# databendlabs/databend

Hardware: AMD Instinct MI355X
Metric: rows/s TPC-H Q1 hash-agg (higher is better)
Workload: dtype i64/i128 decimal

## Files before the change

databend_amd/csrc/gbk_api.h:

```cpp

extern "C" {

int32_t dbhip_group_hash(const dbhip_col* cols, int32_t ncols, int64_t n, uint64_t* out_hashes,
                         void* stream) {
  DBHIP_REQUIRE(cols && ncols >= 1 && ncols <= GB_MAX_KEYS, "dbhip_group_hash: bad column list");
  if (n == 0) return DBHIP_OK;
  DBHIP_REQUIRE(out_hashes, "dbhip_group_hash: NULL out");
  HashCols hc;
  hc.n = ncols;
  for (int k = 0; k < ncols; ++k) {
    if (!key_type_ok(cols[k].type)) {
      set_error("dbhip_group_hash: unsupported type %d", cols[k].type);
      return DBHIP_ERR_INVALID;
    }
    hc.c[k] = to_gbcol(cols[k]);
  }
  hipStream_t s = resolve_stream(stream);
  unsigned long long* bad = (unsigned long long*)scratch(8, 2, s);
  if (!bad) return DBHIP_ERR_HIP;
  DBHIP_CHECK(hipMemsetAsync(bad, 0, 8, s));
  hipLaunchKernelGGL(group_hash_kernel, dim3(grid_for(ceil_div(n, 4), 256, 1024)), dim3(256), 0, s, hc, n, out_hashes, bad);
  DBHIP_LAUNCH_CHECK();
  return DBHIP_OK;
}
// ... 3 lines not shown
                             int64_t initial_capacity, dbhip_groupby** out_host) {
  DBHIP_REQUIRE(out_host && key_types_host, "dbhip_groupby_create: NULL argument");
  dbhip_groupby* g = new (std::nothrow) dbhip_groupby();
  DBHIP_REQUIRE(g, "dbhip_groupby_create: out of host memory");
  memset(g, 0, sizeof(*g));
  int32_t rc = build_layout(key_types_host, key_nullable_host, nkeys, aggs_host, naggs, &g->L);
  if (rc) { delete g; return rc; }
  int64_t cap = 1024;
  while (cap < initial_capacity) cap <<= 1;
  g->hash_mask = ~0ULL;
  g->part_min_rows = 262144;
  g->hint_groups = initial_capacity;
  if (layout_has_wide_minmax(g->L)) { g->part_forbidden = 1; g->part_bits = -1; }
  hipStream_t s = resolve_stream(nullptr);
  if ((rc = alloc_table(g, cap, s))) { delete g; return rc; }
  hipError_t e = hipMalloc((void**)&g->ctrl, 128);
  if (e == hipSuccess) e = hipMemsetAsync(g->ctrl, 0, 128, s);
  if (e == hipSuccess) e = hipStreamSynchronize(s);
  if (e != hipSuccess) {
    (void)dbhip_groupby_destroy(g);
    return hip_fail(e, "dbhip_groupby_create");
  }
  *out_host = g;
  return DBHIP_OK;
}

int32_t dbhip_groupby_debug_set_hash_mask(dbhip_groupby* g, uint64_t mask) {
  DBHIP_REQUIRE(g && g->count_host == 0, "dbhip_groupby_debug_set_hash_mask: table must be empty");
  g->hash_mask = mask;
  return DBHIP_OK;
}

int32_t dbhip_groupby_debug_set_partition_bits(dbhip_groupby* g, int32_t bits) {
  DBHIP_REQUIRE(g && bits <= PT_MAX_BITS, "dbhip_groupby_debug_set_partition_bits: bad argument");
  if (bits > 0) { g->part_bits = bits; g->part_min_rows = 1; g->part_forbidden = 0; }
  else if (bits == 0) { g->part_bits = 0; g->part_min_rows = 262144; g->part_forbidden = 0; }
  else { g->part_bits = -1; g->part_forbidden = 1; g->part_min_rows = 262144; }
// ... 578 lines not shown
  hipLaunchKernelGGL(gb_compact_blocks_kernel, dim3(n_blocks), dim3(256), 0, s, blocks, stride, W, -1, g->rows_in);
  DBHIP_LAUNCH_CHECK();
  return merge_rows(g, g->rows_in, total, s);
}

int32_t dbhip_groupby_reset(dbhip_groupby* g, void* stream) {
  DBHIP_REQUIRE(g, "dbhip_groupby_reset: NULL argument");
  hipStream_t s = resolve_stream(stream);
  if (g->fa_pipe) { const int32_t rc = dbhip_fagg_pipe_reset_internal(g->fa_pipe, s); if (rc) return rc; }
  if (g->cap <= (1 << 20)) {
    hipLaunchKernelGGL(gb_reset_unless_off_kernel, dim3(grid_for(g->cap, 256, 256)), dim3(256), 0, s, (const uint64_t*)nullptr, (int64_t)0, 0, (int64_t)0,
                       g->slot_hash, g->cap, g->ctrl);
    DBHIP_LAUNCH_CHECK();
  } else {
    DBHIP_CHECK(hipMemsetAsync(g->slot_hash, 0, (size_t)g->cap * 8, s));
    DBHIP_CHECK(hipMemsetAsync(g->ctrl, 0, 128, s));
  }
  reset_host_state(g);
  return DBHIP_OK;
}

int32_t dbhip_groupby_destroy(dbhip_groupby* g) {
  if (!g) return DBHIP_OK;
  (void)hipDeviceSynchronize();
  if (g->fa_pipe) dbhip_fagg_pipe_destroy_internal(g->fa_pipe);
  if (g->slot_hash) (void)dbhip_free(g->slot_hash);
  if (g->rows) (void)dbhip_free(g->rows);
  if (g->ctrl) (void)hipFree(g->ctrl);
  if (g->rows_in) (void)dbhip_free(g->rows_in);
  if (g->gid) (void)dbhip_free(g->gid);
  if (g->retry) (void)dbhip_free(g->retry);
  if (g->partial) (void)dbhip_free(g->partial);
  if (g->part_meta) (void)dbhip_free(g->part_meta);
  if (g->spill_idx) (void)dbhip_free(g->spill_idx);
  if (g->spill_rows) (void)dbhip_free(g->spill_rows);
  if (g->gbc_spill) (void)dbhip_free(g->gbc_spill);
  if (g->gbc_split) (void)dbhip_free(g->gbc_split);
  if (g->xcur) (void)hipFree(g->xcur);
  if (g->arena) (void)dbhip_free(g->arena);
  delete g;
  return DBHIP_OK;
}

// ... 3 lines not shown
```

databend_amd/csrc/gbk_merge_lds.h:

```cpp

namespace {

int32_t ensure(void** p, size_t* cap, size_t bytes) {
  if (*cap >= bytes) return DBHIP_OK;
  if (*p) {
    int32_t rc = dbhip_free(*p);
    if (rc) return rc;
    *p = nullptr; *cap = 0;
  }
  size_t want = bytes + (bytes >> 3) + 256;
  int32_t rc = dbhip_alloc(want, p);
  if (rc) { *p = nullptr; return rc; }
  *cap = want;
  return DBHIP_OK;
}

int32_t alloc_table(dbhip_groupby* g, int64_t cap, hipStream_t s) {
  uint64_t* nh = nullptr;
  uint64_t* nr = nullptr;
  int32_t rc = dbhip_alloc((size_t)cap * 8, (void**)&nh);
  if (rc == DBHIP_OK) rc = dbhip_alloc((size_t)cap * g->L.W * 8, (void**)&nr);
  hipError_t e = rc == DBHIP_OK ? hipMemsetAsync(nh, 0, (size_t)cap * 8, s) : hipSuccess;
  if (rc != DBHIP_OK || e != hipSuccess) {
    if (nh) (void)dbhip_free(nh);
// ... 163 lines not shown
                            const uint64_t* n_dev, const uint64_t* abort_dev, int deferred) {
  if (n == 0) return DBHIP_OK;
  if (n > 0xFFFFFFF0LL) {
    set_error("groupby: more than 2^32 rows in one call");
    return DBHIP_ERR_INVALID;
  }
  int32_t rc;
  if ((rc = ensure((void**)&g->gid, &g->gid_cap, (size_t)n * 4))) return rc;
  if ((rc = ensure((void**)&g->retry, &g->retry_cap, (size_t)n * 4))) return rc;
  const int grid = grid_for(n, 256);
  uint64_t* host_ctrl = pinned_words(0);
  if (!host_ctrl) return DBHIP_ERR_HIP;
  const uint64_t* cur_rows = rows_in;
  int64_t cur_n = n;
  const DevCount dc{n_dev, abort_dev};
  if ((deferred || (g->count_host + n) * 135 <= g->cap * 100) && n <= 256) {
    hipLaunchKernelGGL(gb_merge_small_kernel, dim3(1), dim3(256), 0, s, g->L, cur_rows, cur_n, g->slot_hash, g->rows, g->cap, g->hash_mask, g->gid,
                       g->retry, g->ctrl, dc, g->arena);
    DBHIP_LAUNCH_CHECK();
    if (deferred) return DBHIP_OK;
    DBHIP_CHECK(hipMemcpyAsync(host_ctrl, g->ctrl, 5 * sizeof(uint64_t), hipMemcpyDeviceToHost, s));
    DBHIP_CHECK(hipStreamSynchronize(s));
    g->count_host = (int64_t)host_ctrl[0];
    if (host_ctrl[3] & 2) {
      set_error("groupby: a string key longer than 12 bytes was met; keep the CPU operator for this block");
      return DBHIP_ERR_UNSUPPORTED;
    }
    if (host_ctrl[1]) {
      set_error("groupby: collision chain filled the table during retry; create the table with a larger capacity");
      return DBHIP_ERR_CAPACITY;
    }
    return DBHIP_OK;
  }
  if (deferred || (g->count_host + n) * 135 <= g->cap * 100) {
    DBHIP_CHECK(hipMemsetAsync(&g->ctrl[1], 0, 16, s));
    hipLaunchKernelGGL(gb_probe_kernel, dim3(grid), dim3(256), 0, s, g->L, cur_rows, cur_n, g->slot_hash, g->rows, g->cap,
                       g->hash_mask, g->gid, g->ctrl, dc, g->arena);
    if (deferred == 1 || (!deferred && g->count_host > 0 && g->count_host <= 32 && n <= 65536) || n <= 2048 || layout_has_wide_minmax(g->L))
      hipLaunchKernelGGL(gb_accum_lowcard_kernel, dim3(deferred == 1 && grid > 16 ? 16 : grid), dim3(256), 0, s, g->L, cur_rows, cur_n, g->rows, g->gid, g->retry,
                         g->ctrl, dc, g->arena);
    else
      hipLaunchKernelGGL(gb_accum_kernel, dim3(grid), dim3(256), 0, s, g->L, cur_rows, cur_n, g->rows, g->gid, g->retry, g->ctrl, dc, g->arena);
    hipLaunchKernelGGL(gb_retry_kernel, dim3(1), dim3(64), 0, s, g->L, cur_rows, g->slot_hash, g->rows, g->cap, g->hash_mask,
                       g->gid, g->retry, g->ctrl, g->arena);
    DBHIP_LAUNCH_CHECK();
    if (deferred) return DBHIP_OK;
    DBHIP_CHECK(hipMemcpyAsync(host_ctrl, g->ctrl, 5 * sizeof(uint64_t), hipMemcpyDeviceToHost, s));
    DBHIP_CHECK(hipStreamSynchronize(s));
    g->count_host = (int64_t)host_ctrl[0];
    if (host_ctrl[3] & 2) {
      set_error("groupby: a string key longer than 12 bytes was met; keep the CPU operator for this block");
      return DBHIP_ERR_UNSUPPORTED;
    }
    if (host_ctrl[1]) {
      set_error("groupby: collision chain filled the table during retry; create the table with a larger capacity");
      return DBHIP_ERR_CAPACITY;
    }
    return DBHIP_OK;
  }
// ... 27 lines not shown
    DBHIP_CHECK(hipMemcpyAsync(host_ctrl, g->ctrl, 5 * sizeof(uint64_t), hipMemcpyDeviceToHost, s));
    DBHIP_CHECK(hipStreamSynchronize(s));
    g->count_host = (int64_t)host_ctrl[0];
    if (host_ctrl[3] & 2) {
      set_error("groupby: a string key longer than 12 bytes was met; keep the CPU operator for this block");
      return DBHIP_ERR_UNSUPPORTED;
    }
    if (host_ctrl[1] & 2) {
      set_error("groupby: collision chain filled the table during retry; create the table with a larger capacity");
      return DBHIP_ERR_CAPACITY;
    }
    return DBHIP_OK;
  }
  set_error("groupby: table did not converge after repeated growth");
  return DBHIP_ERR_CAPACITY;
}


constexpr int FK_MAXKW = 4;
constexpr int FK_MAXA = 6;
constexpr uint32_t FK_SPILL = 0xFFFFFFFFu;

template <int KW, int NA, bool HI>
struct FkRow {
  uint64_t kw[KW];
  uint64_t h;
  uint64_t aw[NA];
  uint64_t ah[HI ? NA : 1];
  uint32_t avalid;
};
// ... 246 lines not shown
```

databend_amd/csrc/gbk_partitioned.h:

```cpp

namespace {
__device__ __forceinline__ uint32_t part_of(uint64_t h, int pbits) { return (uint32_t)(h >> (64 - pbits)); }
#include "gb_compact.h"

bool gbc_enabled(const dbhip_groupby* g) {
  return !g->gbc_off && g->hash_mask == ~0ULL && !g->has_long;
}

#define GBC_NV_DISPATCH(KW_, nv_, CALL)                                                                          \
  do { if (nv_ == 1) { CALL(KW_, 1); } else if (nv_ == 2) { CALL(KW_, 2); } else if (nv_ == 4) { CALL(KW_, 4); } else { CALL(KW_, 8); } } while (0)
#define GBC_DISPATCH(D, CALL)                                                     \
  do {                                                                            \
    const int nvc_ = gbc_nv_class(D);                                             \
    switch ((D).kw) {                                                             \
      case 1: GBC_NV_DISPATCH(1, nvc_, CALL); break;                              \
      case 2: GBC_NV_DISPATCH(2, nvc_, CALL); break;                              \
      case 3: GBC_NV_DISPATCH(3, nvc_, CALL); break;                              \
      default: GBC_NV_DISPATCH(4, nvc_, CALL); break;                             \
    }                                                                             \
  } while (0)
#define GBC_FOR_ALL(M) M(1, 1) M(1, 2) M(1, 4) M(1, 8) M(2, 1) M(2, 2) M(2, 4) M(2, 8) M(3, 1) M(3, 2) M(3, 4) M(3, 8) M(4, 1) M(4, 2) M(4, 4) M(4, 8)

constexpr int PT_MAX_BITS = 14;
constexpr int PT_PMAX = 1 << PT_MAX_BITS;
// ... 116 lines not shown
    const int64_t tile_rows = (int64_t)threads * R;
    const int64_t cn = n - *done < limit ? n - *done : limit;
    const int64_t ntiles = ceil_div(cn, tile_rows);
    int grid = (int)(ntiles < max_grid_i ? ntiles : max_grid_i);
    if (!gbc && !g->fast_trusted && ntiles >= 64) {
      const int64_t gmax = probing ? ntiles / 4 : ntiles / 8;
      if (grid > gmax) grid = (int)gmax;
    }
    const int64_t tpb = ceil_div(ntiles, grid);
    grid = (int)ceil_div(ntiles, tpb);
    if ((rc = ensure((void**)&g->partial, &g->partial_cap, (size_t)grid * lcap_i * L.W * 8))) return rc;
    int64_t spill_cap = cn;
    if (g->fast_trusted && cn > (4 << 20)) spill_cap = cn / 64 > (4 << 20) ? cn / 64 : (4 << 20);
    if ((rc = ensure((void**)&g->rows_in, &g->rows_in_cap, (size_t)spill_cap * L.W * 8))) return rc;
    DBHIP_CHECK(hipMemsetAsync(&g->ctrl[5], 0, 16, s));
    FkArgs A;
    A.spill_cap = (uint64_t)spill_cap;
    A.row0 = *done; A.n = cn; A.tiles_per_block = tpb; A.lcap = lcap_i; A.sw = sw;
    A.llimit = (uint32_t)(lcap_i - lcap_i / 4);
    A.hash_mask = g->hash_mask; A.partial = g->partial; A.spill = g->rows_in; A.ctrl = g->ctrl;
    if (gbc) {
      static std::once_flag gbc_attr_once;
      static hipError_t gbc_attr_err = hipSuccess;
      std::call_once(gbc_attr_once, [] {
#define GBC_RAISE(KW_, NV_) if (gbc_attr_err == hipSuccess) gbc_attr_err = hipFuncSetAttribute((const void*)gbc_agg_kernel<KW_, NV_, true>, hipFuncAttributeMaxDynamicSharedMemorySize, 150 * 1024);
        GBC_FOR_ALL(GBC_RAISE)
#undef GBC_RAISE
      });
      DBHIP_CHECK(gbc_attr_err);
      GbcAggArgs G;
// ... 841 lines not shown
    hipLaunchKernelGGL((gb_part_scatter_kernel<2>), dim3((int)nwg), dim3(T), lds2, s, L, C, row0, cn, pbits, rows_per_wg, mat,
                       g->rows_in, g->ctrl);
  else if (lds1 <= lds_max)
    hipLaunchKernelGGL((gb_part_scatter_kernel<1>), dim3((int)nwg), dim3(T), lds1, s, L, C, row0, cn, pbits, rows_per_wg, mat,
                       g->rows_in, g->ctrl);
  else
    hipLaunchKernelGGL((gb_part_scatter_kernel<0>), dim3((int)nwg), dim3(T), (size_t)P * 4, s, L, C, row0, cn, pbits,
                       rows_per_wg, mat, g->rows_in, g->ctrl);
  DBHIP_LAUNCH_CHECK();
  return DBHIP_OK;
}

int32_t add_chunk_partitioned(dbhip_groupby* g, const GbCols& C, int64_t row0, int64_t cn, hipStream_t s,
                              int64_t* spilled) {
  const GbLayout& L = g->L;
  const int pbits = g->part_bits;
  const int P = 1 << pbits;
  int lcap, sw;
  size_t lds_bytes;
  int32_t rc;
  GbcDesc D;
  const bool gbc = g->gbc_active && !g->gbc_skip && !g->part_direct && gbc_enabled(g) && gbc_describe(L, C, &D);
  D.ctrl = g->ctrl;
  if (!gbc) g->gbc_active = 0;
  table_geometry(g, &lcap, &sw, &lds_bytes);
  if (gbc) rc = gbc_partition_scatter(g, C, D, row0, cn, pbits, s);
  else rc = partition_scatter(g, C, row0, cn, pbits, s);
  if (rc) return rc;
  if (!gbc && (rc = ensure((void**)&g->spill_idx, &g->spill_idx_cap, (size_t)cn * 4))) return rc;
  uint32_t* base = g->part_meta + PT_PMAX;
// ... 213 lines not shown
```

databend_amd/csrc/gbk_rows.h:

```cpp

namespace {

struct HashCols {
  GbCol c[GB_MAX_KEYS];
  int n;
};

__global__ __launch_bounds__(256) void group_hash_kernel(HashCols hc, int64_t n, uint64_t* out,
                                                         unsigned long long* bad) {
  constexpr int U = 4;
  const int64_t T = (int64_t)gridDim.x * blockDim.x;
  const int64_t t = (int64_t)blockIdx.x * blockDim.x + threadIdx.x;
  for (int64_t base = 0; base < n; base += U * T) {
    int64_t row[U];
    bool in[U];
    uint64_t h[U];
#pragma unroll
    for (int u = 0; u < U; ++u) {
      row[u] = base + u * T + t;
      in[u] = row[u] < n;
      if (!in[u]) row[u] = n - 1;
      h[u] = 0;
    }
    for (int k = 0; k < hc.n; ++k) {
// ... 450 lines not shown
        for (int a = 0; a < L.naggs; ++a) gb_atomic_merge(L, a, d + L.agg_off[a], r + L.agg_off[a]);
        done = true;
      }
      pos = (pos + 1) & cmask;
    }
    if (!done) ctrl[1] |= 2;
  }
}
__global__ void gb_retry_kernel(GbLayout L, const uint64_t* rows_in, uint64_t* slot_hash, uint64_t* rows,
                                int64_t cap, uint64_t hash_mask, const uint32_t* gid,
                                const uint32_t* retry, uint64_t* ctrl, uint8_t* arena) {
  if (threadIdx.x != 0 || blockIdx.x != 0) return;
  gb_retry_body(L, rows_in, slot_hash, rows, cap, hash_mask, gid, retry, ctrl, arena);
}

__global__ __launch_bounds__(256) void gb_merge_small_kernel(GbLayout L, const uint64_t* rows_in, int64_t n, uint64_t* slot_hash, uint64_t* rows,
                                                             int64_t cap, uint64_t hash_mask, uint32_t* gid, uint32_t* retry, uint64_t* ctrl,
                                                             DevCount dc, uint8_t* arena) {
  n = dev_rows(dc, n);
  if (threadIdx.x < 2) ctrl[1 + threadIdx.x] = 0;
  __threadfence();
  __syncthreads();
  gb_probe_body(L, rows_in, n, slot_hash, rows, cap, hash_mask, gid, ctrl, arena);
  __threadfence();
  __syncthreads();
  gb_accum_lowcard_body(L, rows_in, n, rows, gid, retry, ctrl, arena);
  __threadfence();
  __syncthreads();
  if (threadIdx.x == 0) gb_retry_body(L, rows_in, slot_hash, rows, cap, hash_mask, gid, retry, ctrl, arena);
}

__global__ __launch_bounds__(256) void gb_rehash_kernel(GbLayout L, const uint64_t* old_hash,
                                                        const uint64_t* old_rows, int64_t old_cap,
                                                        uint64_t* new_hash, uint64_t* new_rows,
                                                        int64_t new_cap, uint64_t hash_mask) {
  const uint64_t cmask = (uint64_t)new_cap - 1;
  for (int64_t s = (int64_t)blockIdx.x * blockDim.x + threadIdx.x; s < old_cap;
       s += (int64_t)gridDim.x * blockDim.x) {
    uint64_t hw = old_hash[s];
    if (hw == 0) continue;
    const uint64_t* r = old_rows + s * L.W;
    uint64_t pos = home_slot(probe_word(r[L.hash_word], hash_mask), new_cap);
    while (true) {
      unsigned long long old = atomicCAS((unsigned long long*)&new_hash[pos], 0ULL, (unsigned long long)hw);
// ... 71 lines not shown
  uint64_t off = 0;
  for (int p = 0; p < b; ++p)
    if (p != skip) off += blocks[(int64_t)p * stride_words];
  const uint64_t* src = blocks + (int64_t)b * stride_words + W;
  uint64_t* dst = out + off * W;
  for (uint64_t i = threadIdx.x; i < cnt * (uint64_t)W; i += blockDim.x) dst[i] = src[i];
}

__global__ __launch_bounds__(256) void gb_reset_unless_off_kernel(const uint64_t* __restrict__ blocks, int64_t stride_words, int n_blocks,
                                                                  int64_t max_rows, uint64_t* __restrict__ slot_hash, int64_t cap, uint64_t* __restrict__ ctrl) {
  for (int p = 0; p < n_blocks; ++p) {
    const uint64_t c = blocks[(int64_t)p * stride_words];
    if (c == ~0ULL || (int64_t)c > max_rows || blocks[(int64_t)p * stride_words + 1] != 0) return;
  }
  for (int64_t i = (int64_t)blockIdx.x * blockDim.x + threadIdx.x; i < cap; i += (int64_t)gridDim.x * blockDim.x) slot_hash[i] = 0;
  if (blockIdx.x == 0 && threadIdx.x < 16) ctrl[threadIdx.x] = 0;
}

struct ResultPtrs {
  void* keys[GB_MAX_KEYS];
  uint32_t* key_validity[GB_MAX_KEYS];
  void* aggs[GB_MAX_AGGS];
  uint32_t* agg_validity[GB_MAX_AGGS];
  uint64_t* hashes;
  const uint8_t* arena;
};

__device__ __forceinline__ bool gb_sum256_out_of_range(const uint64_t* s) {
  const bool neg = (s[3] >> 63) != 0;
  if (s[4] != (neg ? ~0ULL : 0ULL)) return true;
  uint64_t m[4] = {s[0], s[1], s[2], s[3]};
// ... 399 lines not shown
```

databend_amd/csrc/k_fagg.hip:

```cpp
#include "fagg_device.h"
#include "runtime.h"

#include <dirent.h>
#include <dlfcn.h>
#include <errno.h>
#include <sys/stat.h>
#include <fcntl.h>
#include <signal.h>
#include <spawn.h>
#include <sys/wait.h>
#include <unistd.h>

#include <atomic>
#include <chrono>
#include <deque>
#include <map>
#include <mutex>
#include <string>

#include <stdlib.h>
#include <string.h>
#include <time.h>

using namespace dbhip;

int32_t dbhip_groupby_merge_rows_dev_internal(dbhip_groupby* g, const uint64_t* rows, int64_t n_max, const uint64_t* n_dev,
                                              const uint64_t* abort_dev, hipStream_t s);
int32_t dbhip_groupby_merge_rows_internal(dbhip_groupby* g, const uint64_t* rows, int64_t n, hipStream_t s);
int64_t dbhip_groupby_capacity_internal(dbhip_groupby* g);
int32_t dbhip_groupby_reserve_merge_internal(dbhip_groupby* g, int64_t n);
int64_t dbhip_groupby_count_internal(dbhip_groupby* g);
const GbLayout* dbhip_groupby_layout_internal(dbhip_groupby* g);
int32_t dbhip_groupby_merge_rows_deferred_internal(dbhip_groupby* g, const uint64_t* rows, int64_t n_max, const uint64_t* n_dev,
                                                   const uint64_t* abort_dev, hipStream_t s);
int32_t dbhip_groupby_ensure_room_internal(dbhip_groupby* g, int64_t extra, hipStream_t s);
uint64_t* dbhip_groupby_ctrl_internal(dbhip_groupby* g);
void dbhip_groupby_set_count_internal(dbhip_groupby* g, int64_t count);
void** dbhip_groupby_pipe_slot_internal(dbhip_groupby* g);

namespace {

#include "build/jit_embed.inc"
// ... 898 lines not shown
  if (rc) return rc;
  A.filter_bits = filter_bitmap; A.filter_off = filter_bit_offset; A.n = n;
  A.has_filter = filter_bitmap != nullptr;
  const size_t lds = (size_t)(A.P.n_slots > 6 ? A.P.n_slots : 6) * FA_ROWS * 256 * 8;
  if (lds > 60 * 1024) {
    set_error("dbhip_groupby_add_block_program: %d live LDS slots exceed the register file; split the expression", A.P.n_slots);
    return DBHIP_ERR_UNSUPPORTED;
  }
  const int64_t nchunks = ceil_div(n, 64 * FA_ROWS);
  const int grid = (int)(ceil_div(nchunks, 4) < 512 ? ceil_div(nchunks, 4) : 512);
  if (FaPipe* pp = (FaPipe*)*dbhip_groupby_pipe_slot_internal(g); pp && !t_prepare_only) {
    int64_t committed = 0;
    if ((rc = fa_pipe_checkpoint(g, pp, &committed, true))) return rc;
  }
  const size_t rows_bytes = (size_t)grid * FA_MAX_SLOTS * L.W * 8;
  uint8_t* ws = (uint8_t*)scratch(rows_bytes + 64, 6, s);
  if (!ws) return DBHIP_ERR_HIP;
  uint64_t* ctrl = (uint64_t*)ws;
  A.ctrl = ctrl;
  A.partial_rows = (uint64_t*)(ws + 64);
  A.P.err_words = nullptr;
  A.P.err_count = (unsigned long long*)&ctrl[2];
  uint64_t* host_ctrl = pinned_words(1);
  if (!host_ctrl) return DBHIP_ERR_HIP;
  host_ctrl[0] = host_ctrl[1] = host_ctrl[2] = 0;
  const int64_t n_max = (int64_t)grid * FA_MAX_SLOTS;
  const bool chained = (dbhip_groupby_count_internal(g) + n_max) * 135 <= dbhip_groupby_capacity_internal(g) * 100;
  if ((rc = dbhip_groupby_reserve_merge_internal(g, n_max))) return rc;
  if (t_prepare_only) {
    (void)jit_kernel(A, dbhip_groupby_count_internal(g) > 4 ? 8 : 4, general, nwords, JIT_COMPILE);
    if (FaPipe* pq = (FaPipe*)*dbhip_groupby_pipe_slot_internal(g); pq && pq->on)
      (void)jit_kernel(A, dbhip_groupby_count_internal(g) > 4 ? 8 : 4, general, nwords, JIT_COMPILE, nullptr, true);
    return DBHIP_OK;
  }
  for (int variant = dbhip_groupby_count_internal(g) > 4 ? 1 : 0; variant < 2; ++variant) {
    DBHIP_CHECK(hipMemsetAsync(ctrl, 0, 64, s));
    kernel_timer_start(s);
    if ((rc = fa_launch(A, variant == 0 ? 4 : 8, general, nwords, grid, lds, s))) return rc;
    kernel_timer_stop(s);
    DBHIP_LAUNCH_CHECK();
    DBHIP_CHECK(hipMemcpyAsync(host_ctrl, ctrl, 24, hipMemcpyDeviceToHost, s));
    if (chained && !may_raise) {
      rc = dbhip_groupby_merge_rows_dev_internal(g, A.partial_rows, n_max, &ctrl[0], &ctrl[1], s);
      if (rc) return rc;
      if (!(host_ctrl[1] & 3)) return DBHIP_OK;
    } else {
      DBHIP_CHECK(hipStreamSynchronize(s));
    }
    if (!(host_ctrl[1] & 1)) break;
  }
  if (host_ctrl[1] & 2) {
    set_error("dbhip_groupby_add_block_program: a group key string is longer than 12 bytes");
    return DBHIP_ERR_UNSUPPORTED;
  }
  if (host_ctrl[1] & 1) {
    set_error("dbhip_groupby_add_block_program: more than %d distinct groups inside one workgroup; use the operator-at-a-time path", FA_MAX_SLOTS);
    return DBHIP_ERR_CAPACITY;
  }
  if (host_ctrl[2]) {
    set_error("dbhip_groupby_add_block_program: %llu row error(s) in the fused maps (Decimal overflow / divided by zero); "
              "evaluate the maps with dbhip_expr_eval to get the rows", (unsigned long long)host_ctrl[2]);
    return DBHIP_ERR_ROW_ERRORS;
  }
// ... 105 lines not shown
      if (inputs[c].data == col.data && inputs[c].type == col.type && inputs[c].validity == col.validity &&
          inputs[c].validity_offset == col.validity_offset && inputs[c].is_scalar == col.is_scalar) found = c;
    if (found < 0) {
      if (n_inputs >= EX_MAX_INPUTS) return DBHIP_ERR_UNSUPPORTED;
      if (col.type == DBHIP_T_DEC128) { int wide = 0; for (int c = 0; c < n_inputs; ++c) wide += inputs[c].type == DBHIP_T_DEC128; if (wide >= 2) return DBHIP_ERR_UNSUPPORTED; }
      inputs[n_inputs] = col;
      found = n_inputs++;
    }
    arg_regs[a] = DBHIP_ARG_INPUT(found);
    any_arg = true;
  }
  if (!any_arg) return DBHIP_ERR_UNSUPPORTED;
  dbhip_agg_program prog;
  prog.prog = nullptr; prog.n_ins = 0; prog.inputs = inputs; prog.n_inputs = n_inputs; prog.filter_reg = -1; prog.arg_regs = arg_regs;
  t_jit_only = true; t_jit_pending = false; t_jit_may_compile = may_compile;
  const int32_t rc = dbhip_groupby_add_block_program(g, keys, &prog, n, C.filter, C.filter_off + row0, (void*)s);
  t_jit_only = false;
  return rc;
}
int32_t dbhip_fagg_pipe_add_columns_internal(dbhip_groupby* g, void* pipe, const GbCols& C, int64_t n, hipStream_t s) {
  FaPipe* pp = (FaPipe*)pipe;
  if (!pp || !pp->on || pp->given_up || jit_mode() == 0) return -1;
  const GbLayout& L = *dbhip_groupby_layout_internal(g);
  if (!dbhip_fagg_layout_ok_internal(L)) return -1;
  dbhip_col keys[FA_KW], inputs[EX_MAX_INPUTS];
  int32_t arg_regs[FA_MAXA];
  int n_inputs = 0;
  for (int k = 0; k < L.nkeys; ++k)
    if (!fa_offset_col(C.key[k], 0, &keys[k])) return -1;
  bool any_arg = false;
// ... 74 lines not shown
```

databend_amd/csrc/k_groupby.hip:

```cpp
#include <mutex>
#include "gb_device.h"
#include "runtime.h"

#include <math.h>
#include <stdlib.h>
#include <string.h>

#include <new>
#include <vector>

using namespace dbhip;

#define GB_INVALID_SLOT 0xFFFFFFFFu

struct dbhip_groupby {
  int64_t hint_groups;
  GbLayout L;
  int64_t cap;
  uint64_t* slot_hash;
  uint64_t* rows;
  uint64_t* ctrl;
  uint64_t hash_mask;
  int64_t count_host;
  uint64_t* rows_in; size_t rows_in_cap;
// ... 18 lines not shown
  int has_long;
  uint64_t* xcur;
  int xcur_dirty;
  int fagg_disabled;
  int gbc_off;
  int gbc_active;
  int gbc_lcap;
  int gbc_nodirect;
  int gbc_part_lcap_max;
  uint32_t gbc_part_cap;
  uint64_t* gbc_spill; size_t gbc_spill_cap;
  uint64_t arena_pinned, arena_live;
  int gbc_skip;
  uint32_t* gbc_split; size_t gbc_split_cap;
  void* fa_pipe;
};

int32_t dbhip_fagg_pipe_drain_internal(dbhip_groupby* g, void* pipe, hipStream_t s);
void dbhip_fagg_pipe_destroy_internal(void* pipe);
int32_t dbhip_fagg_pipe_reset_internal(void* pipe, hipStream_t s);
struct GbCols;
int32_t dbhip_fagg_pipe_add_columns_internal(dbhip_groupby* g, void* pipe, const GbCols& C, int64_t n, hipStream_t s);
#define GB_DRAIN(g, s)                                                                   \
  do {                                                                                   \
    if ((g) && (g)->fa_pipe) {                                                           \
      const int32_t _rc = dbhip_fagg_pipe_drain_internal((g), (g)->fa_pipe, (s));        \
      if (_rc) return _rc;                                                               \
    }                                                                                    \
  } while (0)

#include "gbk_rows.h"
int32_t dbhip_groupby_build_layout_internal(const int32_t* key_types, const uint8_t* key_nullable, int nkeys, const dbhip_agg_desc* aggs,
                                            int naggs, GbLayout* L) {
  return build_layout(key_types, key_nullable, nkeys, aggs, naggs, L);
}
#include "gbk_merge_lds.h"
int32_t dbhip_fagg_add_columns_internal(dbhip_groupby* g, const GbCols& C, int64_t row0, int64_t n, bool may_compile, hipStream_t s);
bool dbhip_fagg_last_refusal_is_pending_internal();
#include "gbk_partitioned.h"

int32_t dbhip_groupby_merge_rows_internal(dbhip_groupby* g, const uint64_t* rows, int64_t n, hipStream_t s) {
  return merge_rows(g, rows, n, s);
}
int32_t dbhip_groupby_merge_rows_dev_internal(dbhip_groupby* g, const uint64_t* rows, int64_t n_max, const uint64_t* n_dev,
                                              const uint64_t* abort_dev, hipStream_t s) {
  return merge_rows(g, rows, n_max, s, n_dev, abort_dev);
}
int32_t dbhip_groupby_reserve_merge_internal(dbhip_groupby* g, int64_t n) {
  int32_t rc;
  if ((rc = ensure((void**)&g->gid, &g->gid_cap, (size_t)n * 4))) return rc;
  return ensure((void**)&g->retry, &g->retry_cap, (size_t)n * 4);
}
int32_t dbhip_groupby_merge_rows_deferred_internal(dbhip_groupby* g, const uint64_t* rows, int64_t n_max, const uint64_t* n_dev,
                                                   const uint64_t* abort_dev, hipStream_t s) {
  return merge_rows_unpinned(g, rows, n_max, s, n_dev, abort_dev, 1);
}
int32_t dbhip_groupby_ensure_room_internal(dbhip_groupby* g, int64_t extra, hipStream_t s) {
  uint64_t cnt = 0;
  DBHIP_CHECK(hipMemcpyAsync(&cnt, &g->ctrl[0], 8, hipMemcpyDeviceToHost, s));
  DBHIP_CHECK(hipStreamSynchronize(s));
  g->count_host = (int64_t)cnt;
  while ((g->count_host + extra) * 135 > g->cap * 100) {
// ... 14 lines not shown
```

databend_amd/csrc/k_q1.hip:

```cpp
#include "gb_device.h"
#include "runtime.h"

#include <stdlib.h>
#include <string.h>

using namespace dbhip;

int32_t dbhip_groupby_merge_rows_internal(dbhip_groupby* g, const uint64_t* rows, int64_t n, hipStream_t s);
int32_t dbhip_groupby_merge_rows_dev_internal(dbhip_groupby* g, const uint64_t* rows, int64_t n_max, const uint64_t* n_dev,
                                              const uint64_t* abort_dev, hipStream_t s);
int64_t dbhip_groupby_capacity_internal(dbhip_groupby* g);
int64_t dbhip_groupby_count_internal(dbhip_groupby* g);
const GbLayout* dbhip_groupby_layout_internal(dbhip_groupby* g);

namespace {

constexpr int MAX_SLOTS = 8;
constexpr int Q1_W = 15;

struct alignas(16) U4 {
  uint32_t x, y, z, w;
};
struct alignas(16) L2 {
  int64_t a, b;
};
// ... 282 lines not shown
                   L->key_type[1] == DBHIP_T_STRING && L->agg_off[0] == 5 && L->agg_off[2] == 7 &&
                   L->agg_off[5] == 14 && L->agg_words[2] == 3 && L->agg_words[3] == 3;
  DBHIP_REQUIRE(layout_ok, "dbhip_q1_fused: table was not created by dbhip_q1_create_groupby");
  if (n == 0) return DBHIP_OK;
  DBHIP_REQUIRE(l_quantity && l_extendedprice && l_discount && l_tax && l_returnflag_views &&
                    l_linestatus_views && l_shipdate,
                "dbhip_q1_fused: NULL column");
  uintptr_t al = (uintptr_t)l_quantity | (uintptr_t)l_extendedprice | (uintptr_t)l_discount |
                 (uintptr_t)l_tax | (uintptr_t)l_returnflag_views | (uintptr_t)l_linestatus_views;
  DBHIP_REQUIRE((al & 15) == 0 && ((uintptr_t)l_shipdate & 7) == 0,
                "dbhip_q1_fused: columns must be 16-byte aligned (shipdate 8-byte)");
  hipStream_t s = resolve_stream(stream);
  const int64_t ntiles = ceil_div(n, 128);
  const int grid = (int)(ceil_div(ntiles, 4) < 512 ? ceil_div(ntiles, 4) : 512);
  size_t rows_bytes = (size_t)grid * MAX_SLOTS * Q1_W * 8;
  uint8_t* ws = (uint8_t*)scratch(rows_bytes + 64, 4, s);
  if (!ws) return DBHIP_ERR_HIP;
  uint64_t* ctrl = (uint64_t*)ws;
  uint64_t* partial = (uint64_t*)(ws + 64);
  Q1Args A;
  A.qty = l_quantity; A.price = l_extendedprice; A.disc = l_discount; A.tax = l_tax;
  A.rf = (const U4*)l_returnflag_views; A.ls = (const U4*)l_linestatus_views;
  A.shipdate = l_shipdate; A.cutoff = shipdate_cutoff; A.n = n;
  A.partial_rows = partial; A.ctrl = ctrl;
  uint64_t* host_ctrl = pinned_words(1);
  if (!host_ctrl) return DBHIP_ERR_HIP;
  host_ctrl[0] = host_ctrl[1] = 0;
  const int64_t n_max4 = (int64_t)grid * 4, n_max8 = (int64_t)grid * MAX_SLOTS;
  const bool chained = (dbhip_groupby_count_internal(g) + n_max8) * 135 <= dbhip_groupby_capacity_internal(g) * 100;
  for (int variant = 0; variant < 2; ++variant) {
    DBHIP_CHECK(hipMemsetAsync(ctrl, 0, 64, s));
    kernel_timer_start(s);
    if (variant == 0) hipLaunchKernelGGL(q1_fused_kernel, dim3(grid), dim3(256), 0, s, A);
    else hipLaunchKernelGGL(q1_fused_kernel_8slots, dim3(grid), dim3(256), 0, s, A);
    kernel_timer_stop(s);
    DBHIP_LAUNCH_CHECK();
    DBHIP_CHECK(hipMemcpyAsync(host_ctrl, ctrl, 16, hipMemcpyDeviceToHost, s));
    if (chained) {
      int32_t rc = dbhip_groupby_merge_rows_dev_internal(g, partial, variant == 0 ? n_max4 : n_max8, &ctrl[0], &ctrl[1], s);
      if (rc) return rc;
      if (!(host_ctrl[1] & 3)) return DBHIP_OK;
    } else {
      DBHIP_CHECK(hipStreamSynchronize(s));
    }
    if (!(host_ctrl[1] & 1)) break;
  }
  if (host_ctrl[1] & 2) {
    set_error("dbhip_q1_fused: a group key string is longer than 12 bytes; use the operator-at-a-time path");
    return DBHIP_ERR_UNSUPPORTED;
  }
  if (host_ctrl[1] & 1) {
    set_error("dbhip_q1_fused: more than %d distinct groups inside one workgroup; use the operator-at-a-time path", MAX_SLOTS);
    return DBHIP_ERR_CAPACITY;
  }
  return dbhip_groupby_merge_rows_internal(g, partial, (int64_t)host_ctrl[0], s);
}

}
```

Measured before the change: 91.63 billion.

## Publish fused-merge outcome through mapped host record and skip redundant ctrl memsets

The fused Q1 and fagg paths now keep their control words inside the group-by ctrl block. The closing merge kernel writes the counts and flags into a host-mapped pinned record tagged with a sequence number. This replaces the separate device-to-host memcpy of ctrl words, and the per-call memsets are skipped when the ctrl words are known to be clean after the previous call. The change adds tail_clean bookkeeping on every path that touches ctrl, plus system-scope atomics in the retry kernel. Any path that misses marking the state dirty could leave stale flags behind.

Result: no change. 90.99 billion (median of 2 runs) (-0.7%).

```diff
diff --git a/databend_amd/csrc/gbk_api.h b/databend_amd/csrc/gbk_api.h
--- a/databend_amd/csrc/gbk_api.h
+++ b/databend_amd/csrc/gbk_api.h
@@ -41,13 +41,14 @@
   if (layout_has_wide_minmax(g->L)) { g->part_forbidden = 1; g->part_bits = -1; }
   hipStream_t s = resolve_stream(nullptr);
   if ((rc = alloc_table(g, cap, s))) { delete g; return rc; }
-  hipError_t e = hipMalloc((void**)&g->ctrl, 128);
-  if (e == hipSuccess) e = hipMemsetAsync(g->ctrl, 0, 128, s);
+  hipError_t e = hipMalloc((void**)&g->ctrl, GB_CTRL_WORDS * 8);
+  if (e == hipSuccess) e = hipMemsetAsync(g->ctrl, 0, GB_CTRL_WORDS * 8, s);
   if (e == hipSuccess) e = hipStreamSynchronize(s);
   if (e != hipSuccess) {
     (void)dbhip_groupby_destroy(g);
     return hip_fail(e, "dbhip_groupby_create");
   }
+  g->tail_clean = 1;
   *out_host = g;
   return DBHIP_OK;
 }
@@ -656,8 +657,9 @@
     DBHIP_LAUNCH_CHECK();
   } else {
     DBHIP_CHECK(hipMemsetAsync(g->slot_hash, 0, (size_t)g->cap * 8, s));
-    DBHIP_CHECK(hipMemsetAsync(g->ctrl, 0, 128, s));
-  }
+    DBHIP_CHECK(hipMemsetAsync(g->ctrl, 0, GB_CTRL_WORDS * 8, s));
+  }
+  g->tail_clean = 1;
   reset_host_state(g);
   return DBHIP_OK;
 }
@@ -669,6 +671,7 @@
   if (g->slot_hash) (void)dbhip_free(g->slot_hash);
   if (g->rows) (void)dbhip_free(g->rows);
   if (g->ctrl) (void)hipFree(g->ctrl);
+  if (g->tail_host) (void)hipHostFree(g->tail_host);
   if (g->rows_in) (void)dbhip_free(g->rows_in);
   if (g->gid) (void)dbhip_free(g->gid);
   if (g->retry) (void)dbhip_free(g->retry);
diff --git a/databend_amd/csrc/gbk_merge_lds.h b/databend_amd/csrc/gbk_merge_lds.h
--- a/databend_amd/csrc/gbk_merge_lds.h
+++ b/databend_amd/csrc/gbk_merge_lds.h
@@ -201,9 +201,11 @@
   const uint64_t* cur_rows = rows_in;
   int64_t cur_n = n;
   const DevCount dc{n_dev, abort_dev};
+  const bool closing = deferred == 3;
+  if (!closing) g->tail_clean = 0;
   if ((deferred || (g->count_host + n) * 135 <= g->cap * 100) && n <= 256) {
     hipLaunchKernelGGL(gb_merge_small_kernel, dim3(1), dim3(256), 0, s, g->L, cur_rows, cur_n, g->slot_hash, g->rows, g->cap, g->hash_mask, g->gid,
-                       g->retry, g->ctrl, dc, g->arena);
+                       g->retry, g->ctrl, dc, g->arena, closing ? g->tail_dev : (uint64_t*)nullptr, g->tail_seq);
     DBHIP_LAUNCH_CHECK();
     if (deferred) return DBHIP_OK;
     DBHIP_CHECK(hipMemcpyAsync(host_ctrl, g->ctrl, 5 * sizeof(uint64_t), hipMemcpyDeviceToHost, s));
@@ -220,16 +222,20 @@
     return DBHIP_OK;
   }
   if (deferred || (g->count_host + n) * 135 <= g->cap * 100) {
-    DBHIP_CHECK(hipMemsetAsync(&g->ctrl[1], 0, 16, s));
+    if (!closing) DBHIP_CHECK(hipMemsetAsync(&g->ctrl[1], 0, 16, s));
     hipLaunchKernelGGL(gb_probe_kernel, dim3(grid), dim3(256), 0, s, g->L, cur_rows, cur_n, g->slot_hash, g->rows, g->cap,
                        g->hash_mask, g->gid, g->ctrl, dc, g->arena);
-    if (deferred == 1 || (!deferred && g->count_host > 0 && g->count_host <= 32 && n <= 65536) || n <= 2048 || layout_has_wide_minmax(g->L))
+    if (deferred == 1 || ((!deferred || closing) && g->count_host > 0 && g->count_host <= 32 && n <= 65536) || n <= 2048 || layout_has_wide_minmax(g->L))
       hipLaunchKernelGGL(gb_accum_lowcard_kernel, dim3(deferred == 1 && grid > 16 ? 16 : grid), dim3(256), 0, s, g->L, cur_rows, cur_n, g->rows, g->gid, g->retry,
                          g->ctrl, dc, g->arena);
     else
       hipLaunchKernelGGL(gb_accum_kernel, dim3(grid), dim3(256), 0, s, g->L, cur_rows, cur_n, g->rows, g->gid, g->retry, g->ctrl, dc, g->arena);
-    hipLaunchKernelGGL(gb_retry_kernel, dim3(1), dim3(64), 0, s, g->L, cur_rows, g->slot_hash, g->rows, g->cap, g->hash_mask,
-                       g->gid, g->retry, g->ctrl, g->arena);
+    if (closing)
+      hipLaunchKernelGGL(gb_retry_close_kernel, dim3(1), dim3(64), 0, s, g->L, cur_rows, g->slot_hash, g->rows, g->cap, g->hash_mask,
+                         g->gid, g->retry, g->ctrl, g->arena, g->tail_dev, g->tail_seq);
+    else
+      hipLaunchKernelGGL(gb_retry_kernel, dim3(1), dim3(64), 0, s, g->L, cur_rows, g->slot_hash, g->rows, g->cap, g->hash_mask,
+                         g->gid, g->retry, g->ctrl, g->arena);
     DBHIP_LAUNCH_CHECK();
     if (deferred) return DBHIP_OK;
     DBHIP_CHECK(hipMemcpyAsync(host_ctrl, g->ctrl, 5 * sizeof(uint64_t), hipMemcpyDeviceToHost, s));
@@ -287,6 +293,60 @@
   }
   set_error("groupby: table did not converge after repeated growth");
   return DBHIP_ERR_CAPACITY;
+}
+
+int32_t fused_begin(dbhip_groupby* g, bool chained, hipStream_t s) {
+  if (chained && !g->tail_host) {
+    uint64_t* host = nullptr;
+    uint64_t* dev = nullptr;
+    DBHIP_CHECK(hipHostMalloc((void**)&host, GB_REC_WORDS * sizeof(uint64_t), hipHostMallocMapped));
+    memset(host, 0, GB_REC_WORDS * sizeof(uint64_t));
+    const hipError_t e = hipHostGetDevicePointer((void**)&dev, host, 0);
+    if (e != hipSuccess || !dev) {
+      (void)hipHostFree(host);
+      return hip_fail(e != hipSuccess ? e : hipErrorInvalidValue, "groupby: mapping the outcome record");
+    }
+    g->tail_host = host;
+    g->tail_dev = dev;
+  }
+  if (!g->tail_clean) {
+    DBHIP_CHECK(hipMemsetAsync(&g->ctrl[GB_CTRL_FUSED], 0, 24, s));
+    if (chained) DBHIP_CHECK(hipMemsetAsync(&g->ctrl[1], 0, 16, s));
+  }
+  g->tail_clean = 0;
+  return DBHIP_OK;
+}
+int32_t fused_finish(dbhip_groupby* g, const uint64_t* rows, int64_t n_max, bool chained, hipStream_t s, uint64_t* out) {
+  uint64_t* fused = g->ctrl + GB_CTRL_FUSED;
+  if (!chained) {
+    uint64_t* host = pinned_words(1);
+    if (!host) return DBHIP_ERR_HIP;
+    DBHIP_CHECK(hipMemcpyAsync(host, fused, 24, hipMemcpyDeviceToHost, s));
+    DBHIP_CHECK(hipStreamSynchronize(s));
+    out[0] = host[0]; out[1] = host[1]; out[2] = host[2];
+    return DBHIP_OK;
+  }
+  ++g->tail_seq;
+  int32_t rc = merge_rows_unpinned(g, rows, n_max, s, &fused[0], &fused[1], 3);
+  if (rc) return rc;
+  DBHIP_CHECK(hipStreamSynchronize(s));
+  const uint64_t* rec = g->tail_host;
+  if (__atomic_load_n(&rec[GB_REC_SEQ], __ATOMIC_ACQUIRE) != g->tail_seq) {
+    set_error("groupby: the outcome record of the merge behind a fused kernel is not the one of this call");
+    return DBHIP_ERR_HIP;
+  }
+  g->tail_clean = 1;
+  out[0] = rec[GB_REC_FUSED_ROWS]; out[1] = rec[GB_REC_FUSED_FLAGS]; out[2] = rec[GB_REC_FUSED_ERRORS];
+  g->count_host = (int64_t)rec[GB_REC_COUNT];
+  if (rec[GB_REC_ERROR] & 2) {
+    set_error("groupby: a string key longer than 12 bytes was met; keep the CPU operator for this block");
+    return DBHIP_ERR_UNSUPPORTED;
+  }
+  if (rec[GB_REC_OVERFLOW]) {
+    set_error("groupby: collision chain filled the table during retry; create the table with a larger capacity");
+    return DBHIP_ERR_CAPACITY;
+  }
+  return pin_string_states(g, s);
 }
 
 
diff --git a/databend_amd/csrc/gbk_partitioned.h b/databend_amd/csrc/gbk_partitioned.h
--- a/databend_amd/csrc/gbk_partitioned.h
+++ b/databend_amd/csrc/gbk_partitioned.h
@@ -154,6 +154,7 @@
     if (g->fast_trusted && cn > (4 << 20)) spill_cap = cn / 64 > (4 << 20) ? cn / 64 : (4 << 20);
     if ((rc = ensure((void**)&g->rows_in, &g->rows_in_cap, (size_t)spill_cap * L.W * 8))) return rc;
     DBHIP_CHECK(hipMemsetAsync(&g->ctrl[5], 0, 16, s));
+    g->tail_clean = 0;
     FkArgs A;
     A.spill_cap = (uint64_t)spill_cap;
     A.row0 = *done; A.n = cn; A.tiles_per_block = tpb; A.lcap = lcap_i; A.sw = sw;
@@ -1025,6 +1026,7 @@
 int32_t add_chunk_partitioned(dbhip_groupby* g, const GbCols& C, int64_t row0, int64_t cn, hipStream_t s,
                               int64_t* spilled) {
   const GbLayout& L = g->L;
+  g->tail_clean = 0;
   const int pbits = g->part_bits;
   const int P = 1 << pbits;
   int lcap, sw;
diff --git a/databend_amd/csrc/gbk_rows.h b/databend_amd/csrc/gbk_rows.h
--- a/databend_amd/csrc/gbk_rows.h
+++ b/databend_amd/csrc/gbk_rows.h
@@ -488,9 +488,30 @@
   gb_retry_body(L, rows_in, slot_hash, rows, cap, hash_mask, gid, retry, ctrl, arena);
 }
 
+constexpr int GB_CTRL_WORDS = 32;
+constexpr int GB_CTRL_FUSED = 16;
+enum { GB_REC_COUNT = 0, GB_REC_OVERFLOW, GB_REC_ERROR, GB_REC_FUSED_ROWS, GB_REC_FUSED_FLAGS, GB_REC_FUSED_ERRORS, GB_REC_SEQ, GB_REC_WORDS };
+__device__ __forceinline__ void gb_close_tail(uint64_t* ctrl, uint64_t* rec, uint64_t seq) {
+  const int src[GB_REC_SEQ] = {0, 1, 3, GB_CTRL_FUSED, GB_CTRL_FUSED + 1, GB_CTRL_FUSED + 2};
+#pragma unroll
+  for (int q = 0; q < GB_REC_SEQ; ++q)
+    __hip_atomic_store(&rec[q], __hip_atomic_load(&ctrl[src[q]], __ATOMIC_RELAXED, __HIP_MEMORY_SCOPE_AGENT), __ATOMIC_RELAXED, __HIP_MEMORY_SCOPE_SYSTEM);
+  ctrl[1] = 0; ctrl[2] = 0;
+  ctrl[GB_CTRL_FUSED] = 0; ctrl[GB_CTRL_FUSED + 1] = 0; ctrl[GB_CTRL_FUSED + 2] = 0;
+  __hip_atomic_store(&rec[GB_REC_SEQ], seq, __ATOMIC_RELEASE, __HIP_MEMORY_SCOPE_SYSTEM);
+  __threadfence_system();
+}
+__global__ void gb_retry_close_kernel(GbLayout L, const uint64_t* rows_in, uint64_t* slot_hash, uint64_t* rows,
+                                      int64_t cap, uint64_t hash_mask, const uint32_t* gid,
+                                      const uint32_t* retry, uint64_t* ctrl, uint8_t* arena, uint64_t* rec, uint64_t seq) {
+  if (threadIdx.x != 0 || blockIdx.x != 0) return;
+  gb_retry_body(L, rows_in, slot_hash, rows, cap, hash_mask, gid, retry, ctrl, arena);
+  gb_close_tail(ctrl, rec, seq);
+}
+
 __global__ __launch_bounds__(256) void gb_merge_small_kernel(GbLayout L, const uint64_t* rows_in, int64_t n, uint64_t* slot_hash, uint64_t* rows,
                                                              int64_t cap, uint64_t hash_mask, uint32_t* gid, uint32_t* retry, uint64_t* ctrl,
-                                                             DevCount dc, uint8_t* arena) {
+                                                             DevCount dc, uint8_t* arena, uint64_t* rec = nullptr, uint64_t seq = 0) {
   n = dev_rows(dc, n);
   if (threadIdx.x < 2) ctrl[1 + threadIdx.x] = 0;
   __threadfence();
@@ -501,7 +522,10 @@
   gb_accum_lowcard_body(L, rows_in, n, rows, gid, retry, ctrl, arena);
   __threadfence();
   __syncthreads();
-  if (threadIdx.x == 0) gb_retry_body(L, rows_in, slot_hash, rows, cap, hash_mask, gid, retry, ctrl, arena);
+  if (threadIdx.x == 0) {
+    gb_retry_body(L, rows_in, slot_hash, rows, cap, hash_mask, gid, retry, ctrl, arena);
+    if (rec) gb_close_tail(ctrl, rec, seq);
+  }
 }
 
 __global__ __launch_bounds__(256) void gb_rehash_kernel(GbLayout L, const uint64_t* old_hash,
@@ -603,7 +627,7 @@
     if (c == ~0ULL || (int64_t)c > max_rows || blocks[(int64_t)p * stride_words + 1] != 0) return;
   }
   for (int64_t i = (int64_t)blockIdx.x * blockDim.x + threadIdx.x; i < cap; i += (int64_t)gridDim.x * blockDim.x) slot_hash[i] = 0;
-  if (blockIdx.x == 0 && threadIdx.x < 16) ctrl[threadIdx.x] = 0;
+  if (blockIdx.x == 0 && threadIdx.x < GB_CTRL_WORDS) ctrl[threadIdx.x] = 0;
 }
 
 struct ResultPtrs {
diff --git a/databend_amd/csrc/k_fagg.hip b/databend_amd/csrc/k_fagg.hip
--- a/databend_amd/csrc/k_fagg.hip
+++ b/databend_amd/csrc/k_fagg.hip
@@ -24,8 +24,11 @@
 
 using namespace dbhip;
 
-int32_t dbhip_groupby_merge_rows_dev_internal(dbhip_groupby* g, const uint64_t* rows, int64_t n_max, const uint64_t* n_dev,
-                                              const uint64_t* abort_dev, hipStream_t s);
+uint64_t* dbhip_groupby_fused_ctrl_internal(dbhip_groupby* g);
+int32_t dbhip_groupby_fused_begin_internal(dbhip_groupby* g, bool chained, hipStream_t s);
+int32_t dbhip_groupby_fused_finish_internal(dbhip_groupby* g, const uint64_t* rows, int64_t n_max, bool chained, hipStream_t s,
+                                            uint64_t* out_host);
+void dbhip_groupby_tail_dirty_internal(dbhip_groupby* g);
 int32_t dbhip_groupby_merge_rows_internal(dbhip_groupby* g, const uint64_t* rows, int64_t n, hipStream_t s);
 int64_t dbhip_groupby_capacity_internal(dbhip_groupby* g);
 int32_t dbhip_groupby_reserve_merge_internal(dbhip_groupby* g, int64_t n);
@@ -954,16 +957,14 @@
     if ((rc = fa_pipe_checkpoint(g, pp, &committed, true))) return rc;
   }
   const size_t rows_bytes = (size_t)grid * FA_MAX_SLOTS * L.W * 8;
-  uint8_t* ws = (uint8_t*)scratch(rows_bytes + 64, 6, s);
+  uint8_t* ws = (uint8_t*)scratch(rows_bytes, 6, s);
   if (!ws) return DBHIP_ERR_HIP;
-  uint64_t* ctrl = (uint64_t*)ws;
+  uint64_t* ctrl = dbhip_groupby_fused_ctrl_internal(g);
   A.ctrl = ctrl;
-  A.partial_rows = (uint64_t*)(ws + 64);
+  A.partial_rows = (uint64_t*)ws;
   A.P.err_words = nullptr;
   A.P.err_count = (unsigned long long*)&ctrl[2];
-  uint64_t* host_ctrl = pinned_words(1);
-  if (!host_ctrl) return DBHIP_ERR_HIP;
-  host_ctrl[0] = host_ctrl[1] = host_ctrl[2] = 0;
+  uint64_t host_ctrl[3] = {0, 0, 0};
   const int64_t n_max = (int64_t)grid * FA_MAX_SLOTS;
   const bool chained = (dbhip_groupby_count_internal(g) + n_max) * 135 <= dbhip_groupby_capacity_internal(g) * 100;
   if ((rc = dbhip_groupby_reserve_merge_internal(g, n_max))) return rc;
@@ -973,20 +974,15 @@
       (void)jit_kernel(A, dbhip_groupby_count_internal(g) > 4 ? 8 : 4, general, nwords, JIT_COMPILE, nullptr, true);
     return DBHIP_OK;
   }
+  const bool queued = chained && !may_raise;
   for (int variant = dbhip_groupby_count_internal(g) > 4 ? 1 : 0; variant < 2; ++variant) {
-    DBHIP_CHECK(hipMemsetAsync(ctrl, 0, 64, s));
+    if ((rc = dbhip_groupby_fused_begin_internal(g, queued, s))) return rc;
     kernel_timer_start(s);
     if ((rc = fa_launch(A, variant == 0 ? 4 : 8, general, nwords, grid, lds, s))) return rc;
     kernel_timer_stop(s);
     DBHIP_LAUNCH_CHECK();
-    DBHIP_CHECK(hipMemcpyAsync(host_ctrl, ctrl, 24, hipMemcpyDeviceToHost, s));
-    if (chained && !may_raise) {
-      rc = dbhip_groupby_merge_rows_dev_internal(g, A.partial_rows, n_max, &ctrl[0], &ctrl[1], s);
-      if (rc) return rc;
-      if (!(host_ctrl[1] & 3)) return DBHIP_OK;
-    } else {
-      DBHIP_CHECK(hipStreamSynchronize(s));
-    }
+    if ((rc = dbhip_groupby_fused_finish_internal(g, A.partial_rows, n_max, queued, s, host_ctrl))) return rc;
+    if (queued && !(host_ctrl[1] & 3)) return DBHIP_OK;
     if (!(host_ctrl[1] & 1)) break;
   }
   if (host_ctrl[1] & 2) {
@@ -1122,6 +1118,7 @@
   dbhip_agg_program prog;
   prog.prog = nullptr; prog.n_ins = 0; prog.inputs = inputs; prog.n_inputs = n_inputs; prog.filter_reg = -1; prog.arg_regs = arg_regs;
   t_jit_only = true; t_jit_pending = false; t_jit_may_compile = may_compile;
+  dbhip_groupby_tail_dirty_internal(g);
   const int32_t rc = dbhip_groupby_add_block_program(g, keys, &prog, n, C.filter, C.filter_off + row0, (void*)s);
   t_jit_only = false;
   return rc;
diff --git a/databend_amd/csrc/k_groupby.hip b/databend_amd/csrc/k_groupby.hip
--- a/databend_amd/csrc/k_groupby.hip
+++ b/databend_amd/csrc/k_groupby.hip
@@ -56,6 +56,9 @@
   int gbc_skip;
   uint32_t* gbc_split; size_t gbc_split_cap;
   void* fa_pipe;
+  int tail_clean;
+  uint64_t tail_seq;
+  uint64_t* tail_host; uint64_t* tail_dev;
 };
 
 int32_t dbhip_fagg_pipe_drain_internal(dbhip_groupby* g, void* pipe, hipStream_t s);
@@ -84,10 +87,13 @@
 int32_t dbhip_groupby_merge_rows_internal(dbhip_groupby* g, const uint64_t* rows, int64_t n, hipStream_t s) {
   return merge_rows(g, rows, n, s);
 }
-int32_t dbhip_groupby_merge_rows_dev_internal(dbhip_groupby* g, const uint64_t* rows, int64_t n_max, const uint64_t* n_dev,
-                                              const uint64_t* abort_dev, hipStream_t s) {
-  return merge_rows(g, rows, n_max, s, n_dev, abort_dev);
+uint64_t* dbhip_groupby_fused_ctrl_internal(dbhip_groupby* g) { return g->ctrl + GB_CTRL_FUSED; }
+int32_t dbhip_groupby_fused_begin_internal(dbhip_groupby* g, bool chained, hipStream_t s) { return fused_begin(g, chained, s); }
+int32_t dbhip_groupby_fused_finish_internal(dbhip_groupby* g, const uint64_t* rows, int64_t n_max, bool chained, hipStream_t s,
+                                            uint64_t* out_host) {
+  return fused_finish(g, rows, n_max, chained, s, out_host);
 }
+void dbhip_groupby_tail_dirty_internal(dbhip_groupby* g) { g->tail_clean = 0; }
 int32_t dbhip_groupby_reserve_merge_internal(dbhip_groupby* g, int64_t n) {
   int32_t rc;
   if ((rc = ensure((void**)&g->gid, &g->gid_cap, (size_t)n * 4))) return rc;
diff --git a/databend_amd/csrc/k_q1.hip b/databend_amd/csrc/k_q1.hip
--- a/databend_amd/csrc/k_q1.hip
+++ b/databend_amd/csrc/k_q1.hip
@@ -7,8 +7,10 @@
 using namespace dbhip;
 
 int32_t dbhip_groupby_merge_rows_internal(dbhip_groupby* g, const uint64_t* rows, int64_t n, hipStream_t s);
-int32_t dbhip_groupby_merge_rows_dev_internal(dbhip_groupby* g, const uint64_t* rows, int64_t n_max, const uint64_t* n_dev,
-                                              const uint64_t* abort_dev, hipStream_t s);
+uint64_t* dbhip_groupby_fused_ctrl_internal(dbhip_groupby* g);
+int32_t dbhip_groupby_fused_begin_internal(dbhip_groupby* g, bool chained, hipStream_t s);
+int32_t dbhip_groupby_fused_finish_internal(dbhip_groupby* g, const uint64_t* rows, int64_t n_max, bool chained, hipStream_t s,
+                                            uint64_t* out_host);
 int64_t dbhip_groupby_capacity_internal(dbhip_groupby* g);
 int64_t dbhip_groupby_count_internal(dbhip_groupby* g);
 const GbLayout* dbhip_groupby_layout_internal(dbhip_groupby* g);
@@ -321,35 +323,28 @@
   const int64_t ntiles = ceil_div(n, 128);
   const int grid = (int)(ceil_div(ntiles, 4) < 512 ? ceil_div(ntiles, 4) : 512);
   size_t rows_bytes = (size_t)grid * MAX_SLOTS * Q1_W * 8;
-  uint8_t* ws = (uint8_t*)scratch(rows_bytes + 64, 4, s);
+  uint8_t* ws = (uint8_t*)scratch(rows_bytes, 4, s);
   if (!ws) return DBHIP_ERR_HIP;
-  uint64_t* ctrl = (uint64_t*)ws;
-  uint64_t* partial = (uint64_t*)(ws + 64);
+  uint64_t* ctrl = dbhip_groupby_fused_ctrl_internal(g);
+  uint64_t* partial = (uint64_t*)ws;
   Q1Args A;
   A.qty = l_quantity; A.price = l_extendedprice; A.disc = l_discount; A.tax = l_tax;
   A.rf = (const U4*)l_returnflag_views; A.ls = (const U4*)l_linestatus_views;
   A.shipdate = l_shipdate; A.cutoff = shipdate_cutoff; A.n = n;
   A.partial_rows = partial; A.ctrl = ctrl;
-  uint64_t* host_ctrl = pinned_words(1);
-  if (!host_ctrl) return DBHIP_ERR_HIP;
-  host_ctrl[0] = host_ctrl[1] = 0;
+  uint64_t host_ctrl[3] = {0, 0, 0};
   const int64_t n_max4 = (int64_t)grid * 4, n_max8 = (int64_t)grid * MAX_SLOTS;
   const bool chained = (dbhip_groupby_count_internal(g) + n_max8) * 135 <= dbhip_groupby_capacity_internal(g) * 100;
   for (int variant = 0; variant < 2; ++variant) {
-    DBHIP_CHECK(hipMemsetAsync(ctrl, 0, 64, s));
+    int32_t rc = dbhip_groupby_fused_begin_internal(g, chained, s);
+    if (rc) return rc;
     kernel_timer_start(s);
     if (variant == 0) hipLaunchKernelGGL(q1_fused_kernel, dim3(grid), dim3(256), 0, s, A);
     else hipLaunchKernelGGL(q1_fused_kernel_8slots, dim3(grid), dim3(256), 0, s, A);
     kernel_timer_stop(s);
     DBHIP_LAUNCH_CHECK();
-    DBHIP_CHECK(hipMemcpyAsync(host_ctrl, ctrl, 16, hipMemcpyDeviceToHost, s));
-    if (chained) {
-      int32_t rc = dbhip_groupby_merge_rows_dev_internal(g, partial, variant == 0 ? n_max4 : n_max8, &ctrl[0], &ctrl[1], s);
-      if (rc) return rc;
-      if (!(host_ctrl[1] & 3)) return DBHIP_OK;
-    } else {
-      DBHIP_CHECK(hipStreamSynchronize(s));
-    }
+    if ((rc = dbhip_groupby_fused_finish_internal(g, partial, variant == 0 ? n_max4 : n_max8, chained, s, host_ctrl))) return rc;
+    if (chained && !(host_ctrl[1] & 3)) return DBHIP_OK;
     if (!(host_ctrl[1] & 1)) break;
   }
   if (host_ctrl[1] & 2) {
```
